# Dicklesworthstone/frankensearch

Hardware: AMD Instinct MI355X
Metric: queries/sec + p50 phase-1 latency, 10M×384 f16 corpus, 1/2/4/8 MI355X (higher is better)
Workload: dtype f16 x f32 -> f32 (every emitted score, in the reference's operation order); candidate filter i8 x i8 -> i32

## Files before the change

### frankensearch_amd/_lib.py

```python
from __future__ import annotations

import ctypes as C
import os

HERE = os.path.dirname(os.path.abspath(__file__))
LIB_PATH = os.path.join(HERE, "libfsgpu.so")

OK = 0
ERR_DIMENSION_MISMATCH = 1
ERR_INVALID_CONFIG = 2
ERR_INDEX_CORRUPTED = 3
ERR_INDEX_VERSION_MISMATCH = 4
ERR_IO = 5
ERR_DEVICE = 6
ERR_NO_DEVICE = 7
ERR_NULL_ARGUMENT = 8
ERR_EMBEDDING_FAILED = 9
ERR_MODEL_LOAD_FAILED = 10

ZERO_SIGNAL_NONE = 0
ZERO_SIGNAL_CALLER_REQUESTED_ZERO_K = 1
ZERO_SIGNAL_ZERO_NORM_QUERY = 2
ZERO_SIGNAL_FILTER_ELIMINATED_ALL = 3
ZERO_SIGNAL_NEWLY_CREATED_EMPTY = 4
# ... 86 lines not shown
    "fsgpu_sharded_search_end": (_i32, [_vp, _u64, _vp, _vp, _vp, _vp]),
    "fsgpu_sharded_quant_scale_max": (C.c_float, [_vp]),
    "fsgpu_sharded_set_coalescing": (_i32, [_vp, _u32, _u32]),
    "fsgpu_sharded_coalescing_stats": (_i32, [_vp, C.POINTER(_u64), C.POINTER(_u64)]),
    "fsgpu_sharded_alignment_create": (_i32, [_vp, _vp, C.POINTER(_vp)]),
    "fsgpu_sharded_quality_scores_for_hits": (_i32, [_vp, _vp, _vp, _vp, _u32, _vp, _u32, _vp, _vp]),
    "fsgpu_sharded_open_fsvi": (_i32, [C.c_char_p, _vp, _u32, _i32, C.POINTER(_vp)]),
    "fsgpu_sharded_set_live_bitmap": (_i32, [_vp, _vp]),
    "fsgpu_sharded_soft_delete": (_i32, [_vp, C.c_char_p, _u32, C.POINTER(_i32)]),
    "fsgpu_sharded_wal_append": (_i32, [_vp, C.c_char_p, _u32, _vp, _u32]),
    "fsgpu_sharded_wal_record_count": (_u64, [_vp]),
    "fsgpu_sharded_doc_id": (_i32, [_vp, _u32, C.POINTER(_vp), C.POINTER(_u32)]),
    "fsgpu_sharded_search_hits": (_i32, [_vp, _vp, _u32, _u32, _vp, _vp, C.POINTER(_u32)]),
    "fsgpu_sharded_gather_dot": (_i32, [_vp, _vp, _u32, _vp, _u32, _vp]),
    "fsgpu_search_topk_classified": (_i32, [_vp, _vp, _u32, _u32, _vp, _vp, C.POINTER(_u32), C.POINTER(_i32)]),
    "fsgpu_search_topk_int8_two_pass": (_i32, [_vp, _vp, _u32, _u32, _u32, _vp, _vp, C.POINTER(_u32)]),
    "fsgpu_search_hits": (_i32, [_vp, _vp, _u32, _u32, _vp, _vp, C.POINTER(_u32)]),
    "fsgpu_search_hits_batched": (_i32, [_vp, _vp, _u32, _u32, _u32, _vp, _vp, _vp, C.POINTER(_u32)]),
    "fsgpu_search_hits_batched_device_queries": (_i32, [_vp, _vp, _u32, _u32, _u32, _vp, _vp, _vp, C.POINTER(_u32)]),
    "fsgpu_search_hits_two_pass_batched": (_i32, [_vp, _vp, _u32, _u32, _u32, _u32, _u32, _vp, _vp, _vp, C.POINTER(_u32)]),
    "fsgpu_lab_index_wal_scores": (_i32, [_vp, _vp, _u32, _vp]),
    "fsgpu_gather_dot": (_i32, [_vp, _vp, _u32, _vp, _u32, _vp]),
    "fsgpu_lab_sort_keys_desc": (_i32, [_i32, _vp, _u64, _u64, _vp]),
    "fsgpu_bench_fixture_device": (_i32, [_i32, _u64, _u64, _u32, _u32, C.c_float, _u64, _i32, _vp, _vp]),
    "fsgpu_encode_f32_to_f16": (_i32, [_i32, _vp, _u64, _vp]),
    "fsgpu_widen_f16_to_f32": (_i32, [_i32, _vp, _u64, _vp]),
    "fsgpu_m2v_create": (_i32, [_i32, _vp, _u32, _u32, C.POINTER(_vp)]),
    "fsgpu_m2v_destroy": (None, [_vp]),
    "fsgpu_m2v_dimension": (_u32, [_vp]),
    "fsgpu_m2v_embed": (_i32, [_vp, _vp, _vp, _u32, _vp]),
    "fsgpu_bert_create": (_i32, [_i32, _vp, _vp, C.POINTER(_vp)]),
    "fsgpu_bert_create_safetensors": (_i32, [_i32, _vp, _u64, C.c_float, C.POINTER(_vp)]),
    "fsgpu_bert_create_ex": (_i32, [_i32, _vp, _vp, _vp, C.POINTER(_vp)]),
    "fsgpu_bert_create_safetensors_ex": (_i32, [_i32, _vp, _u64, C.c_float, _vp, C.POINTER(_vp)]),
    "fsgpu_bert_linear_format": (_u32, [_vp]),
    "fsgpu_lab_linear_int8_dynamic": (_i32, [_i32, _vp, _vp, _vp, _u32, _u32, _u32, _vp]),
    "fsgpu_lab_bert_stage": (_i32, [_i32, _vp]),
    "fsgpu_lab_bert_short_stage": (_i32, [_i32, _vp]),
    "fsgpu_bert_destroy": (None, [_vp]),
    "fsgpu_bert_embed_device": (_i32, [_vp, _vp, _vp, _u32, _vp]),
    "fsgpu_m2v_embed_device": (_i32, [_vp, _vp, _vp, _u32, _vp]),
    "fsgpu_search_topk_batched_device_queries": (_i32, [_vp, _vp, _u32, _u32, _u32, _vp, _vp, _vp, C.POINTER(_u32)]),
    "fsgpu_search_topk_int8_two_pass_batched_device_queries": (_i32, [_vp, _vp, _u32, _u32, _u32, _u32, _vp, _vp, _vp, C.POINTER(_u32)]),
    "fsgpu_device_malloc": (_i32, [_i32, _u64, C.POINTER(_vp)]),
    "fsgpu_device_free": (_i32, [_i32, _vp]),
    "fsgpu_bert_device": (_i32, [_vp]),
# ... 127 lines not shown
```

### frankensearch_amd/csrc/fsgpu_api.cpp

```cpp
#include "../../include/fsgpu.h"
#include "../../include/fsgpu_lab.h"

#include <algorithm>
#include <cmath>
#include <cstring>
#include <exception>
#include <limits>
#include <new>
#include <string>
#include <vector>

#include <atomic>
#include <mutex>
#include <shared_mutex>

#include "bert_embedder.hpp"
#include "bert_reranker.hpp"
#include "coalescer.hpp"
#include "index_builder.hpp"
#include "sharded_index.hpp"
#include "vector_index.hpp"
#include "two_tier_index.hpp"

struct CoalescedCall : fsgpu::CoalescedRequest {
// ... 1625 lines not shown
    return guarded([&]() -> fsgpu_status {
        int count = 0;
        if (hipGetDeviceCount(&count) != hipSuccess || count <= 0) return fail(FSGPU_ERR_NO_DEVICE, "no HIP device visible");
        if (device < 0 || device >= count) return fail(FSGPU_ERR_INVALID_CONFIG, "device ordinal out of range");
        if (hipSetDevice(device) != hipSuccess) return fail(FSGPU_ERR_DEVICE, "hipSetDevice failed");
        if (n == 0) return FSGPU_OK;
        fsgpu::DeviceBuffer in, out, tmp;
        size_t tmp_bytes = 0;
        (void)fsgpu::sort_keys_desc_temp_bytes(n, &tmp_bytes);
        fsgpu::SearchError e = in.reserve(n * 8);
        if (e.ok()) e = out.reserve(n * 8);
        if (e.ok()) e = tmp.reserve(tmp_bytes);
        hipError_t he = hipSuccess;
        if (e.ok()) {
            he = hipMemcpy(in.ptr, keys, n * 8, hipMemcpyHostToDevice);
            if (he == hipSuccess)
                he = fsgpu::sort_keys_desc(tmp.ptr, tmp.bytes, static_cast<const fsgpu::u64*>(in.ptr), static_cast<fsgpu::u64*>(out.ptr), n, nullptr, varying_bits);
            if (he == hipSuccess) he = hipStreamSynchronize(nullptr);
            if (he == hipSuccess) he = hipMemcpy(out_sorted, out.ptr, n * 8, hipMemcpyDeviceToHost);
        }
        in.release();
        out.release();
        tmp.release();
        if (!e.ok()) return finish(e);
        if (he != hipSuccess) return fail(FSGPU_ERR_DEVICE, hipGetErrorString(he));
        return FSGPU_OK;
    });
}

fsgpu_status fsgpu_encode_f32_to_f16(int32_t device, const float* src, uint64_t n, uint16_t* dst) {
    return convert_on_device(device, src, 4, n, dst, 2, true);
}

fsgpu_status fsgpu_widen_f16_to_f32(int32_t device, const uint16_t* src, uint64_t n, float* dst) {
    return convert_on_device(device, src, 2, n, dst, 4, false);
}

fsgpu_status fsgpu_m2v_create(int32_t device, const float* table, uint32_t vocab, uint32_t dim, fsgpu_m2v** out) {
    if (!out) return fail(FSGPU_ERR_NULL_ARGUMENT, "out is null");
    *out = nullptr;
    return guarded([&]() -> fsgpu_status {
        auto* h = new fsgpu_m2v();
        fsgpu::SearchError e = h->impl.init(device, table, vocab, dim);
        if (!e.ok()) {
            delete h;
            return finish(e);
// ... 868 lines not shown
```

### frankensearch_amd/csrc/kernels.hpp

```cpp
#pragma once

#include <hip/hip_runtime.h>
#include <stddef.h>
#include <stdint.h>

namespace fsgpu {

typedef unsigned long long u64;

struct ScanArgs {
    const void* slab;
    const u64* live;
    const u64* allow;
    const float* queries;
    u64* partial;
    uint32_t nrows;
    uint32_t dim;
    uint32_t k;
    uint32_t row_base;
    int32_t hreduce;
    uint32_t row_stride;
};

struct MergeArgs {
// ... 141 lines not shown
constexpr uint32_t kSelectPool = 1024;
constexpr uint32_t kSelectMaxK = 128;
hipError_t launch_select(const SelectArgs& args, int nq, hipStream_t stream);
hipError_t launch_list_cut(const u64* lists, uint32_t nlists, uint32_t list_len, float* out, hipStream_t stream);
hipError_t launch_two_pass_merge(const u64* approx_lists, const u64* exact_lists, uint32_t nshards, uint64_t shard_pitch, uint32_t nq,
                                 uint32_t cc, uint32_t k, uint32_t out_stride, uint32_t* out_rows, float* out_scores, uint32_t* out_counts,
                                 hipStream_t stream);
hipError_t launch_prepare_queries_i8(const float* q, uint32_t nq, uint32_t nq_pad, uint32_t dim, void* qi8, float* delta,
                                     hipStream_t stream, int bits = 8);
hipError_t launch_prepare_queries_i8_filter(const float* q, uint32_t nq, uint32_t nq_pad, uint32_t dim, uint32_t q_stride,
                                            const unsigned int* slab_max_bits, const unsigned int* slab_stats, void* qi8,
                                            float* delta, hipStream_t stream, float* unit_out = nullptr, double extra_coeff = 0.0);

constexpr uint32_t kMfmaMaxSlots = 32;
constexpr uint32_t kMfmaSpillCountStride = 16;
constexpr uint32_t kWideSlots = 32;
bool scan_mfma_supported(int dim);
bool scan_wide_supported(int dim, int elem_bytes);
bool scan_wide_group_maxima_supported(int dim, int query_tiles);
int scan_wide_max_query_tiles(int dim, int elem_bytes);
hipError_t launch_scan_wide(const MfmaScanArgs& args, int query_tiles, int grid, hipStream_t stream, int* occupancy);
void note_main_pass_kernel(const char* name);
const char* last_main_pass_kernel();
int scan_mfma_waves_per_block(int shape);
int scan_mfma_rows_per_tile(int shape);
int scan_mfma_query_tiles(int shape);
int scan_mfma_max_slots(int shape);
hipError_t launch_scan_mfma(const MfmaScanArgs& args, int shape, int grid, hipStream_t stream, int* occupancy);
hipError_t launch_max_row_norm(const void* slab, uint32_t nrows, uint32_t dim, uint32_t row_stride_bytes, unsigned int* out_bits,
                               hipStream_t stream);
hipError_t launch_prepare_queries(const float* q, uint32_t nq, uint32_t nq_pad, uint32_t dim, uint32_t q_stride,
                                  const unsigned int* max_norm_bits, void* qh, float* delta, hipStream_t stream);

hipError_t launch_slab_maxabs(const void* slab_f16, size_t n_values, unsigned int* max_bits_dev, hipStream_t stream);
hipError_t launch_quantize_slab_i8(const void* slab_f16, size_t n_values, unsigned int* max_bits_dev, void* out_i8,
                                   hipStream_t stream, bool max_ready = false);
hipError_t launch_quantize_slab_4bit_levels(const void* slab_f16, size_t n_values, unsigned int* max_bits_dev, void* out_i8,
                                            hipStream_t stream, bool max_ready = false);
hipError_t launch_i8_slab_stats(const void* slab_f16, const void* slab_i8, uint32_t nrows, uint32_t dim,
                                const unsigned int* max_bits_dev, unsigned int* stats_dev, hipStream_t stream);
hipError_t launch_rotate_rows_f16(const void* rows_f16, uint32_t nrows, uint32_t dim, const double* rt, float* out, hipStream_t stream);
hipError_t launch_rotate_rows_f32(const float* rows, uint32_t nrows, uint32_t row_stride, uint32_t dim, const double* rt, float* out,
                                  hipStream_t stream);
hipError_t launch_maxabs_f32(const float* v, size_t n, unsigned int* max_bits_dev, hipStream_t stream);
hipError_t launch_quantize_f32_i8(const float* v, size_t n, const unsigned int* max_bits_dev, void* out_i8, hipStream_t stream);
hipError_t launch_i8_stats_f32(const float* rows, const void* rows_i8, uint32_t nrows, uint32_t dim, const unsigned int* max_bits_dev,
// ... 282 lines not shown
```

### frankensearch_amd/csrc/mfma_scan.hip

```cpp
#include <atomic>
#include <cstdlib>
#include <string>
#include <type_traits>

#include "scan_common.hpp"

namespace fsgpu {

using namespace scan_detail;

typedef float f32x4 __attribute__((ext_vector_type(4)));

template <int DIM_E, int NQT, int WPB, int STAGE, int RT, bool PF, int EB = 2>
__global__ __launch_bounds__(WPB * 64) void scan_mfma_kernel(MfmaScanArgs args) {
    constexpr int DIM = DIM_E * EB / 2;
    typedef int i32x4 __attribute__((ext_vector_type(4)));
    using acc_t = std::conditional_t<EB == 2, f32x4, i32x4>;
    constexpr int NT = WPB * 64;
    constexpr int KS = DIM / 32;
    constexpr int QSTRIDE = DIM + 16;
    constexpr int NQ = NQT * 16;
    extern __shared__ __attribute__((aligned(16))) unsigned char smem[];
    _Float16* qs = reinterpret_cast<_Float16*>(smem);
    const int tid = threadIdx.x, lane = tid & 63;
// ... 256 lines not shown
}
template <int KL>
__device__ __forceinline__ void merge_wave_winners(const u64* win, int k, u64* top, int lane) {
    static_assert(KL == 1, "ranks up to 64");
    if (k <= 16) merge_wave_winners_e<4>(win, k, top, lane);
    else if (k <= 32) merge_wave_winners_e<8>(win, k, top, lane);
    else merge_wave_winners_e<kSelWaves>(win, k, top, lane);
}

constexpr int kSelSortCap = 8192;
constexpr int kRescoreBatch = 6;
constexpr int kSelQueryLds = 1024;
#ifdef FSGPU_EXPERIMENTS
#define SEL_STAMP(slot)                                                                                            \
    do {                                                                                                             \
        if (args.stamps && (blockIdx.x & 255) == 0 && blockIdx.x < 1024 && threadIdx.x == 0)                    \
            args.stamps[(blockIdx.x >> 8) * 16 + (slot)] = (unsigned long long)clock64();                              \
    } while (0)
#else
#define SEL_STAMP(slot) \
    do {                \
    } while (0)
#endif
template <bool FINISH, bool SORTED>
__global__ __launch_bounds__(kSelThreads, SORTED ? 4 : kSelMinWaves) void select_kernel(SelectArgs args) {
    constexpr int NT = kSelThreads, PER = kSelPer, NW = kSelWaves, POOL = (int)kSelectPool, KL = 1;
    static_assert(POOL == NT, "one pool entry per thread in the final selection");
    __shared__ u64 win[2][NW * 64 * KL];
    __shared__ u64 top[64 * KL];
    extern __shared__ __attribute__((aligned(16))) unsigned char sel_dyn[];
    u64* sbuf = reinterpret_cast<u64*>(sel_dyn);
    __shared__ u64 pool[POOL];
    __shared__ int s_count;
    __shared__ float s_tau;
    __shared__ u64 s_gmax[64];
    __shared__ __attribute__((aligned(16))) float s_q[FINISH ? kSelQueryLds : 4];
    __shared__ int s_quick;
    __shared__ u64 s_kth[2];
    const int tid = threadIdx.x, lane = tid & 63, wave = tid >> 6;
    const int q = blockIdx.x;
    SEL_STAMP(0);
    if (args.big_pool && args.pool_flag && args.pool_flag[q] == 0) return;
    auto reset_spill = [&]() {
        if (tid == 0 && args.spill_reset) args.spill_reset[(size_t)q * kMfmaSpillCountStride] = 0u;
    };
    const int k = (int)args.k;
// ... 54 lines not shown
            if (!have) e[x] = kEmpty;
            if (i < lists32) {
                const uint32_t l = i / args.list_len, j = i - l * args.list_len;
                const bool in_list = !cnts || j < (l < kSelCntCap ? s_cnt[l] : cnts[l]);
                if (have && j < kSpecSlots) {
                    if (!in_list) e[x] = kEmpty;
                } else if (in_list) {
                    e[x] = in[(size_t)l * args.l_stride + j];
                } else {
                    e[x] = kEmpty;
                }
            } else if (i < extra_end) {
                e[x] = args.extra[(size_t)q * args.extra_len + (i - lists32)];
            } else if (i < total32) {
                e[x] = args.spill[(size_t)q * args.spill_cap + (i - extra_end)];
            } else {
                e[x] = kEmpty;
            }
        }
    };
    if (tid == 0) s_count = 0;
    pool[tid] = kEmpty;
    int ncand = 0;
    if constexpr (SORTED) {
        __syncthreads();
        for (int p = 0; p < npass; ++p) {
            load_pass(p, e);
#pragma unroll
            for (int x = 0; x < PER; ++x) {
                const bool ok = e[x] != kEmpty;
                const u64 m = __ballot(ok);
                if (m) {
                    int wbase = 0;
                    if (lane == 0) wbase = atomicAdd(&s_count, (int)__popcll(m));
                    wbase = __shfl(wbase, 0);
                    const int pos = wbase + (int)__popcll(m & ((1ull << lane) - 1ull));
                    if (ok && pos < kSelSortCap) sbuf[pos] = e[x];
                }
            }
        }
        __syncthreads();
        int cnt = s_count;
        if (cnt > kSelSortCap) {
            if (tid == 0 && args.overflow) args.overflow[q] = 1;
            cnt = kSelSortCap;
        }
        int np2 = 64;
// ... 466 lines not shown
    if (occupancy) {
        int blocks = 0;
        if (hipOccupancyMaxActiveBlocksPerMultiprocessor(&blocks, kern, WPB * 64, lds) != hipSuccess || blocks < 1) blocks = 1;
        *occupancy = blocks;
        return hipSuccess;
    }
    if (STAGE == 2) {
        static const std::string name = "scan_mfma_kernel<" + std::to_string(DIM) + ", " + std::to_string(NQT) + ", " +
                                        std::to_string(WPB) + ", " + std::to_string(STAGE) + ", " + std::to_string(RT) + ", " +
                                        (PF ? "true" : "false") + ", " + std::to_string(EB) + ">";
        g_last_main_pass_kernel.store(name.c_str(), std::memory_order_relaxed);
    }
    hipLaunchKernelGGL(kern, dim3(grid, args.groups ? args.groups : 1), dim3(WPB * 64), lds, stream, args);
    return hipGetLastError();
}

template <int DIM, int NQT, int WPB, int RT, bool PF, int EB>
static hipError_t launch_mfma_t(const MfmaScanArgs& args, int grid, hipStream_t stream, int* occupancy) {
    if (args.stage == 0) return launch_mfma_s<DIM, NQT, WPB, 0, 1, true, EB>(args, grid, stream, occupancy);
    if (args.stage == 1) return launch_mfma_s<DIM, NQT, WPB, 1, RT, PF, EB>(args, grid, stream, occupancy);
    return launch_mfma_s<DIM, NQT, WPB, 2, RT, PF, EB>(args, grid, stream, occupancy);
}

int scan_mfma_waves_per_block(int shape) { return shape == 0 || shape == 3 ? 4 : 8; }
int scan_mfma_rows_per_tile(int shape) { return shape == 4 ? 64 : (shape >= 2 ? 32 : 16); }
int scan_mfma_query_tiles(int shape) { return shape == 0 ? 4 : (shape == 5 ? 10 : 8); }
int scan_mfma_max_slots(int shape) { return shape == 5 ? 16 : (int)kMfmaMaxSlots; }

template <int DIM, int EB>
static hipError_t launch_mfma_d(const MfmaScanArgs& args, int shape, int grid, hipStream_t stream, int* occupancy) {
    switch (shape) {
        case 0: return launch_mfma_t<DIM, 4, 4, 1, true, EB>(args, grid, stream, occupancy);
        case 2: return launch_mfma_t<DIM, 8, 8, 2, false, EB>(args, grid, stream, occupancy);
#ifdef FSGPU_EXPERIMENTS
        case 1: return launch_mfma_t<DIM, 8, 8, 1, true, EB>(args, grid, stream, occupancy);
        case 3: return launch_mfma_t<DIM, 8, 4, 2, true, EB>(args, grid, stream, occupancy);
        case 4:
            if constexpr (EB == 1) return launch_mfma_t<DIM, 8, 8, 4, false, EB>(args, grid, stream, occupancy);
            return hipErrorInvalidValue;
        case 5: return launch_mfma_t<DIM, 10, 8, 2, false, EB>(args, grid, stream, occupancy);
#endif
        default: return hipErrorInvalidValue;
    }
}

hipError_t launch_scan_mfma(const MfmaScanArgs& args, int shape, int grid, hipStream_t stream, int* occupancy) {
// ... 88 lines not shown
    uint32_t n = 0;
    for (uint32_t j = (uint32_t)tid; j < out_stride; j += 256) {
        const u64 v = j < k && j < (uint32_t)np2 && akey[j] != 0 ? aval[j] : kEmpty;
        if (out_rows) out_rows[(size_t)q * out_stride + j] = (uint32_t)v;
        if (out_scores) out_scores[(size_t)q * out_stride + j] = __uint_as_float((uint32_t)(v >> 32));
    }
    if (tid == 0 && out_counts) {
        const uint32_t lim = k < (uint32_t)np2 ? k : (uint32_t)np2;
        while (n < lim && akey[n] != 0) ++n;
        out_counts[q] = n;
    }
}

hipError_t launch_two_pass_merge(const u64* approx_lists, const u64* exact_lists, uint32_t nshards, uint64_t shard_pitch, uint32_t nq,
                                 uint32_t cc, uint32_t k, uint32_t out_stride, uint32_t* out_rows, float* out_scores, uint32_t* out_counts,
                                 hipStream_t stream) {
    if (nq == 0) return hipSuccess;
    if (cc == 0 || (uint64_t)nshards * cc > 1024 || k > cc) return hipErrorInvalidValue;
    hipLaunchKernelGGL(two_pass_merge_kernel, dim3(nq), dim3(256), 0, stream, approx_lists, exact_lists, nshards, shard_pitch, nq, cc, k,
                       out_stride, out_rows, out_scores, out_counts);
    return hipGetLastError();
}

template <bool RANK, int M, int KCAP>
__global__ __launch_bounds__(512) void select_groups_kernel(GroupSelectArgs args) {
    constexpr int NT = 512, NW = NT / 64, PERT = 1024 / NT, PERW = RANK ? KCAP / 4 : 8, W0 = NW * PERW / 64, NR = M * 8;
    static_assert(NR <= 256 && NR <= NT && NW * PERW % 64 == 0 && W0 >= 1, "W0 winners per lane of wave 0; the rank loop runs on NR threads");
    static_assert(M <= 64 && KCAP >= 64 && KCAP % 64 == 0 && (RANK || M <= NW * PERW), "wave 0 picks M (or k <= KCAP) of the waves' winners");
    __shared__ u64 win[NW * PERW];
    __shared__ u64 top[KCAP];
    __shared__ u64 pool[256];
    __shared__ u64 keys[256];
    __shared__ __attribute__((aligned(16))) float s_q[kSelQueryLds];
    __shared__ u64 s_kth;
    const int tid = threadIdx.x, lane = tid & 63, wave = tid >> 6;
    const int q = blockIdx.x;
    const int k = (int)args.k;
    const float d = args.delta[q];
    const bool real_query = args.valid_queries == 0 || (uint32_t)q < args.valid_queries;
    const int dim = (int)args.dim;
    if (real_query) {
        const float* qsrc = args.queries + (size_t)q * (args.query_stride ? args.query_stride : args.dim);
        for (int i = tid; i < dim && i < kSelQueryLds; i += NT) s_q[i] = qsrc[i];
    }
    u64 e[PERT], key[PERT];
#pragma unroll
    for (int x = 0; x < PERT; ++x) {
        const uint32_t i = (uint32_t)tid + (uint32_t)x * NT;
        e[x] = i < args.nentries ? args.groups[(size_t)q * args.nentries + i] : kEmpty;
        key[x] = e[x] != kEmpty ? sortkey(e[x]) : 0ull;
    }
    if (lane < PERW) win[wave * PERW + lane] = kEmpty;
    if (tid < 256) pool[tid] = kEmpty;
    if (tid == 0) s_kth = 0ull;
    wave_lds_fence();
    wave_extract_topk<PERT>(key, e, PERW, win + wave * PERW);
    __syncthreads();
    if (wave == 0) {
        u64 e2[W0], key2[W0];
#pragma unroll
        for (int x = 0; x < W0; ++x) {
            e2[x] = win[lane + 64 * x];
            key2[x] = e2[x] != kEmpty ? sortkey(e2[x]) : 0ull;
        }
#pragma unroll
        for (int x = 0; x < KCAP / 64; ++x) top[lane + 64 * x] = kEmpty;
        wave_lds_fence();
        wave_extract_topk<W0>(key2, e2, RANK ? (k < KCAP ? k : KCAP) : M, top);
        wave_lds_fence();
    }
    __syncthreads();
    if constexpr (RANK) {
        if (tid == 0) {
            float t = -INFINITY;
            if (d < 0.f || !real_query) {
                t = INFINITY;
                if (args.overflow) args.overflow[q] = 1;
            } else if (k <= KCAP && top[k - 1] != kEmpty) {
                const float ta = __uint_as_float((uint32_t)(top[k - 1] >> 32)) - 2.0f * d;
                if (ta == ta) t = ta;
            }
            args.tau_out[q] = t;
            if (args.spill_reset) args.spill_reset[(size_t)q * kMfmaSpillCountStride] = 0u;
        }
        return;
    }
    for (int c0 = 0; c0 < NR; c0 += NT / 4) {
        const int c = c0 + (tid >> 2), a = tid & 3;
        const int gi = c >> 3, pos = c & 7;
        const u64 ge = c < NR ? top[gi] : kEmpty;
        const uint32_t grow = (uint32_t)ge + (uint32_t)((pos >> 2) * 16 + (pos & 3));
        uint32_t row = grow - args.row_base;
        bool mine = real_query && ge != kEmpty && row < args.nrows && dim <= kSelQueryLds;
        if (mine && args.live) mine = ((args.live[row >> 6] >> (row & 63)) & 1ull) != 0;
        if (mine && args.allow) mine = ((args.allow[row >> 6] >> (row & 63)) & 1ull) != 0;
        if (!mine) row = 0;
        const u32x4* p = reinterpret_cast<const u32x4*>(reinterpret_cast<const unsigned char*>(args.slab) + (size_t)row * ((size_t)dim * 2));
        float acc[8];
#pragma unroll
        for (int j = 0; j < 8; ++j) acc[j] = 0.f;
        const int chunks = dim >> 3, groups = chunks >> 2, leftover = chunks & 3;
        for (int g0 = 0; g0 < groups; g0 += kRescoreBatch) {
            u32x4 w[kRescoreBatch];
#pragma unroll
            for (int j = 0; j < kRescoreBatch; ++j)
                if (g0 + j < groups) w[j] = p[4 * (g0 + j) + a];
#pragma unroll
            for (int j = 0; j < kRescoreBatch; ++j)
                if (g0 + j < groups) {
// ... 33 lines not shown
            if (ak != kEmpty) {
                const float ta = __uint_as_float((uint32_t)(ak >> 32)) - 2.0f * d;
                if (ta == ta) t = ta;
            }
            const u64 kth = s_kth;
            if (kth != 0ull) {
                const float sk = __uint_as_float((uint32_t)(kth >> 32));
                const float v = sk * args.anchor_unit[q];
                const float te = v - d - fabsf(v) * 1e-6f - 1.0f;
                if (te == te && te > t) t = te;
            }
        }
        args.tau_out[q] = t;
        if (args.spill_reset) args.spill_reset[(size_t)q * kMfmaSpillCountStride] = 0u;
    }
}

hipError_t launch_select_groups(const GroupSelectArgs& args, int nq, hipStream_t stream) {
    if (args.k < 1 || args.nentries == 0 || args.nentries > 1024 || !args.delta || !args.tau_out) return hipErrorInvalidValue;
    if (args.rank_only ? args.k > kGroupsRankMax : (args.k > kGroupsTakenMax || (args.dim & 7) || args.dim > kSelQueryLds || !args.anchor_unit || !args.slab))
        return hipErrorInvalidValue;
    constexpr int M0 = (int)kGroupsTaken, M1 = (int)kGroupsTakenMax;
    if (args.rank_only) {
        if (args.k <= 64) hipLaunchKernelGGL((select_groups_kernel<true, M0, 64>), dim3(nq), dim3(512), 0, stream, args);
        else hipLaunchKernelGGL((select_groups_kernel<true, M0, (int)kGroupsRankMax>), dim3(nq), dim3(512), 0, stream, args);
    } else {
        if (args.k <= kGroupsTaken) hipLaunchKernelGGL((select_groups_kernel<false, M0, 64>), dim3(nq), dim3(512), 0, stream, args);
        else hipLaunchKernelGGL((select_groups_kernel<false, M1, 64>), dim3(nq), dim3(512), 0, stream, args);
    }
    return hipGetLastError();
}

__global__ __launch_bounds__(256) void list_cut_kernel(const u64* __restrict__ lists, uint32_t nlists, uint32_t list_len, float* __restrict__ out) {
    __shared__ u64 red[4];
    const int tid = threadIdx.x, lane = tid & 63, wave = tid >> 6;
    u64 m = 0;
    for (uint32_t l = tid; l < nlists; l += 256) {
        const u64 e = lists[(size_t)l * list_len + list_len - 1];
        const u64 key = e != kEmpty ? sortkey(e) : 0ull;
        m = key > m ? key : m;
    }
#pragma unroll
    for (int off = 32; off > 0; off >>= 1) {
        const u64 o = __shfl_xor(m, off);
        m = o > m ? o : m;
    }
    if (lane == 0) red[wave] = m;
    __syncthreads();
    if (tid == 0) {
#pragma unroll
        for (int w = 1; w < 4; ++w) m = red[w] > m ? red[w] : m;
// ... 10 lines not shown
hipError_t launch_select(const SelectArgs& args, int nq, hipStream_t stream) {
    if (args.k < 1 || args.k > kSelectMaxK || !args.delta || (uint64_t)args.nlists * args.list_len > 0x7fffffffull)
        return hipErrorInvalidValue;
#ifdef FSGPU_EXPERIMENTS
    static const int sort_above = [] {
        const char* e = std::getenv("FSGPU_SELECT_SORT_ABOVE");
        return e ? std::atoi(e) : 32;
    }();
#else
    constexpr int sort_above = 32;
#endif
    const bool sorted = (int)args.k > sort_above || args.k > 64 || (args.big_pool && args.slab && !args.take_topk);
    constexpr size_t sort_lds = (size_t)kSelSortCap * 8;
    static bool attr_done = false;
    if (!attr_done) {
        hipError_t e1 = hipFuncSetAttribute(reinterpret_cast<const void*>(select_kernel<true, true>),
                                            hipFuncAttributeMaxDynamicSharedMemorySize, (int)sort_lds);
        hipError_t e2 = hipFuncSetAttribute(reinterpret_cast<const void*>(select_kernel<false, true>),
                                            hipFuncAttributeMaxDynamicSharedMemorySize, (int)sort_lds);
        if (e1 != hipSuccess) return e1;
        if (e2 != hipSuccess) return e2;
        attr_done = true;
    }
    if (args.slab) {
        if (args.k_out < 1 || args.k_out > 64 || (args.dim & 7)) return hipErrorInvalidValue;
        if (sorted) hipLaunchKernelGGL((select_kernel<true, true>), dim3(nq), dim3(kSelThreads), sort_lds, stream, args);
        else hipLaunchKernelGGL((select_kernel<true, false>), dim3(nq), dim3(kSelThreads), 0, stream, args);
    } else {
        if (sorted) hipLaunchKernelGGL((select_kernel<false, true>), dim3(nq), dim3(kSelThreads), sort_lds, stream, args);
        else hipLaunchKernelGGL((select_kernel<false, false>), dim3(nq), dim3(kSelThreads), 0, stream, args);
    }
    return hipGetLastError();
}

hipError_t launch_max_row_norm(const void* slab, uint32_t nrows, uint32_t dim, uint32_t row_stride_bytes, unsigned int* out_bits,
                               hipStream_t stream) {
    hipError_t e = hipMemsetAsync(out_bits, 0, 4, stream);
    if (e != hipSuccess) return e;
    hipLaunchKernelGGL(max_row_norm_kernel, dim3(2048), dim3(256), 0, stream, static_cast<const unsigned short*>(slab),
                       nrows, dim, row_stride_bytes ? row_stride_bytes / 2 : dim, out_bits);
    return hipGetLastError();
}

hipError_t launch_prepare_queries(const float* q, uint32_t nq, uint32_t nq_pad, uint32_t dim, uint32_t q_stride,
                                  const unsigned int* max_norm_bits, void* qh, float* delta, hipStream_t stream) {
    hipLaunchKernelGGL(prepare_queries_kernel, dim3(nq_pad), dim3(256), 0, stream, q, nq, q_stride ? q_stride : dim, dim, max_norm_bits,
                       static_cast<_Float16*>(qh), delta);
    return hipGetLastError();
}

}
```

### frankensearch_amd/csrc/vector_index_batched.cpp

```cpp
#include "vector_index.hpp"

#include <algorithm>
#include <cmath>
#include <cstdio>
#include <cstdlib>
#include <chrono>
#include <cstring>
#include <type_traits>

#include "../../include/fsgpu.h"
#include "lab_env.hpp"
#include "vector_index_internal.hpp"

namespace fsgpu {

using namespace detail;

SearchError VectorIndex::search_top_k_batched_device(const float* queries_dev, uint32_t nq, uint32_t query_len,
                                                     uint32_t k, const uint64_t* allow_dev, uint32_t* out_rows_dev,
                                                     float* out_scores_dev, uint32_t* out_counts_dev,
                                                     hipStream_t stream, uint32_t* fallbacks, uint64_t* out_packed_dev) {
    const bool strided = row_stride_ && row_stride_ != dim_ * 2;
    bool i8f = batched_filter != 1 && (batched_filter == 2 || !i8f_disabled_) && !f32_ && !strided && variant == 0 && knobs().filter != 1 &&
               scan_mfma_supported((int)dim_) && k >= 1 && k <= 64 && nrows_ >= 4 * 8192ull;
// ... 505 lines not shown
        FSGPU_TRY(i8_max_.reserve(4));
        FSGPU_HIP(launch_quantize_slab_i8(slab_dev_, (size_t)nrows_ * dim_, static_cast<unsigned int*>(i8_max_.ptr),
                                          i8_slab_.ptr, stream, quant_max_ready_));
        i8_ready_ = true;
    }
    if (!p.i8 && !mf_norm_ready_) {
        FSGPU_TRY(mf_max_norm_.reserve(4));
        FSGPU_HIP(launch_max_row_norm(slab_dev_, p.N, dim_, p.strided ? row_stride_ : 0, static_cast<unsigned int*>(mf_max_norm_.ptr), stream));
        mf_norm_ready_ = true;
    }
    constexpr uint32_t GMAX = BatchedPlan::GMAX, SPILL = BatchedPlan::SPILL, KC = BatchedPlan::KC;
    const uint32_t round_cap = knobs().round >= (int)GMAX ? (uint32_t)knobs().round : 1024;
    const uint32_t QCAP = std::min<uint32_t>(round_cap, std::max<uint32_t>(std::max<uint32_t>(GMAX, 256), (nq + 127) / 128 * 128));
    p.QCAP = QCAP;
    FSGPU_TRY(mf_qh_.reserve((size_t)QCAP * dim_ * 2));
    FSGPU_TRY(mf_delta_.reserve(QCAP * 4));
    FSGPU_TRY(mf_tau_.reserve(QCAP * 16));
    FSGPU_TRY(mf_spill_.reserve((size_t)QCAP * SPILL * 8 + (size_t)QCAP * kMfmaSpillCountStride * 4));
    FSGPU_TRY(mf_dense_.reserve((size_t)QCAP * RA_MAX * 8));
    FSGPU_TRY(mf_sel_.reserve((size_t)QCAP * KC * 8));
    if (mf_shape_ < 0) {
        mf_shape_ = 2;
        if (knobs().mfma_shape) mf_shape_ = knobs().mfma_shape;
        if (mf_shape_ < 1 || mf_shape_ > 3) mf_shape_ = 2;
        MfmaScanArgs probe{};
        probe.dim = dim_;
        probe.stage = 2;
        FSGPU_HIP(launch_scan_mfma(probe, 0, 1, stream, &mf_per_cu_narrow_));
        FSGPU_HIP(launch_scan_mfma(probe, mf_shape_, 1, stream, &mf_per_cu_wide_));
        probe.elem_bytes = 1;
        mf_shape_i8_ = 2;
        if (knobs().mfma_shape_i8) mf_shape_i8_ = knobs().mfma_shape_i8;
        if (mf_shape_i8_ < 1 || mf_shape_i8_ > 4) mf_shape_i8_ = 2;
        FSGPU_HIP(launch_scan_mfma(probe, 0, 1, stream, &mf_per_cu_narrow_i8_));
        FSGPU_HIP(launch_scan_mfma(probe, mf_shape_i8_, 1, stream, &mf_per_cu_wide_i8_));
        mf_use_160_ = knobs().use_160;
        if (mf_use_160_) {
            FSGPU_HIP(launch_scan_mfma(probe, 5, 1, stream, &mf_per_cu_160_i8_));
            probe.elem_bytes = 2;
            FSGPU_HIP(launch_scan_mfma(probe, 5, 1, stream, &mf_per_cu_160_));
        }
    }
    p.wide_pref = knobs().wide >= 0 ? knobs().wide : 3;
    p.wide_max = (uint32_t)std::max(2, std::min(knobs().wide_max > 0 ? knobs().wide_max : 5, scan_wide_max_query_tiles((int)dim_, p.i8 ? 1 : 2)));
    p.wide_ok = (p.wide_pref == 2 || p.wide_pref == 3) && scan_wide_supported((int)dim_, p.i8 ? 1 : 2) && variant != 5 && variant != 6;
    const uint32_t flag_cap = (nq + GMAX - 1) / GMAX * GMAX + 256;
    if (flag_cap > mf_flags_cap_) {
        if (async_state_[0] == 1 || async_state_[1] == 1)
            return make_error(FSGPU_ERR_INVALID_CONFIG, "a begun batched search is outstanding: end it before searching with a larger batch");
        if (mf_flags_host_) (void)hipHostFree(mf_flags_host_);
        mf_flags_host_ = nullptr;
        mf_flags_cap_ = 0;
        FSGPU_HIP(hipHostMalloc(reinterpret_cast<void**>(&mf_flags_host_), (size_t)flag_cap * 8 * 3, hipHostMallocMapped));
        mf_flags_cap_ = flag_cap;
    }
    uint32_t* flags_area = mf_flags_host_ + (size_t)((async_want_ >= 0 && !hard_batch_) ? 1 + async_want_ : 0) * mf_flags_cap_ * 2;
// ... 663 lines not shown
```

### include/fsgpu_lab.h

```cpp
#ifndef FSGPU_LAB_H
#define FSGPU_LAB_H

#include "fsgpu.h"

#ifdef __cplusplus
extern "C" {
#endif

fsgpu_status fsgpu_bench_fixture_device(int32_t device, uint64_t first, uint64_t n, uint32_t dim, uint32_t clusters, float noise,
                                        uint64_t seed_base, int32_t as_f16, void *out_dev, void *hip_stream);

fsgpu_status fsgpu_index_set_profiling(fsgpu_index *idx, int32_t enabled);
fsgpu_status fsgpu_index_scan_time(fsgpu_index *idx, double *total_ms, uint64_t *launches, int32_t reset);
fsgpu_status fsgpu_index_scan_stats(fsgpu_index *idx, double *total_ms, uint64_t *launches, uint64_t *rows,
                                    int32_t reset);
fsgpu_status fsgpu_index_filter_stats(fsgpu_index *idx, uint64_t *gathered, uint64_t *scanned);
const char *fsgpu_last_main_pass_kernel(void);
fsgpu_status fsgpu_lab_sort_keys_desc(int32_t device, const uint64_t *keys, uint64_t n, uint64_t varying_bits, uint64_t *out_sorted);
fsgpu_status fsgpu_lab_linear_int8_dynamic(int32_t device, const float *x, const float *w, const float *bias, uint32_t m, uint32_t n,
                                           uint32_t k, float *y);
#define FSGPU_LAB_BERT_ATTENTION 0
#define FSGPU_LAB_BERT_LINEAR 1
#define FSGPU_LAB_BERT_LINEAR_LN 2
#define FSGPU_LAB_BERT_POST_ATTN 3
#define FSGPU_LAB_BERT_EMBED_LN 4
#define FSGPU_LAB_BERT_POOL 5
typedef struct fsgpu_lab_bert_stage_args {
    uint32_t stage, form, epilogue;
    uint32_t m, n, k, hidden, inter, n_docs, vocab, max_pos;
    float eps, scale;
    const uint32_t *offsets;
    const int32_t *ids, *positions, *types;
    const float *in[12];
    float *out0, *out1;
} fsgpu_lab_bert_stage_args;
fsgpu_status fsgpu_lab_bert_stage(int32_t device, const fsgpu_lab_bert_stage_args *args);
#define FSGPU_LAB_BERT_Q_ATTN 0
#define FSGPU_LAB_BERT_Q_GEMM 1
#define FSGPU_LAB_BERT_Q_POOL 2
#define FSGPU_LAB_BERT_DOCS 3
typedef struct fsgpu_lab_bert_short_args {
// ... 26 lines not shown
```

Baseline: 366,500.

## Replace sorted top-k selection and group rank threshold with LDS radix select

Adds a byte-wise radix-select path to the sorted select kernel for small candidate sets. It finds the k-th key via 256-bin histograms, compacts the survivors and ranks them, replacing the multi-pass sort and the large dynamic shared-memory allocation. The rank-only group select kernel likewise computes its threshold by radix histogram instead of wave top-k extraction, which removes the KCAP template variant. It also adds a lab test entry point and a guard against MFMA shapes that were not compiled. The trade-off is more barriers and shared-memory atomics in exchange for less sorting work and lower shared-memory use.

```diff
diff --git a/frankensearch_amd/_lib.py b/frankensearch_amd/_lib.py
--- a/frankensearch_amd/_lib.py
+++ b/frankensearch_amd/_lib.py
@@ -132,6 +132,7 @@
     "fsgpu_lab_index_wal_scores": (_i32, [_vp, _vp, _u32, _vp]),
     "fsgpu_gather_dot": (_i32, [_vp, _vp, _u32, _vp, _u32, _vp]),
     "fsgpu_lab_sort_keys_desc": (_i32, [_i32, _vp, _u64, _u64, _vp]),
+    "fsgpu_lab_select_topk": (_i32, [_i32, _vp, _u32, _u32, _u32, _vp]),
     "fsgpu_bench_fixture_device": (_i32, [_i32, _u64, _u64, _u32, _u32, C.c_float, _u64, _i32, _vp, _vp]),
     "fsgpu_encode_f32_to_f16": (_i32, [_i32, _vp, _u64, _vp]),
     "fsgpu_widen_f16_to_f32": (_i32, [_i32, _vp, _u64, _vp]),
diff --git a/frankensearch_amd/csrc/fsgpu_api.cpp b/frankensearch_amd/csrc/fsgpu_api.cpp
--- a/frankensearch_amd/csrc/fsgpu_api.cpp
+++ b/frankensearch_amd/csrc/fsgpu_api.cpp
@@ -1671,6 +1671,48 @@
         in.release();
         out.release();
         tmp.release();
+        if (!e.ok()) return finish(e);
+        if (he != hipSuccess) return fail(FSGPU_ERR_DEVICE, hipGetErrorString(he));
+        return FSGPU_OK;
+    });
+}
+
+fsgpu_status fsgpu_lab_select_topk(int32_t device, const uint64_t* entries, uint32_t nq, uint32_t n, uint32_t k, uint64_t* out) {
+    if (nq && (!out || (n && !entries))) return fail(FSGPU_ERR_NULL_ARGUMENT, "entries / out is null");
+    if (n > 8192 || k < 1 || k > 128) return fail(FSGPU_ERR_INVALID_CONFIG, "n <= 8192, 1 <= k <= 128");
+    return guarded([&]() -> fsgpu_status {
+        int count = 0;
+        if (hipGetDeviceCount(&count) != hipSuccess || count <= 0) return fail(FSGPU_ERR_NO_DEVICE, "no HIP device visible");
+        if (device < 0 || device >= count) return fail(FSGPU_ERR_INVALID_CONFIG, "device ordinal out of range");
+        if (hipSetDevice(device) != hipSuccess) return fail(FSGPU_ERR_DEVICE, "hipSetDevice failed");
+        if (nq == 0) return FSGPU_OK;
+        constexpr size_t POOL = fsgpu::kSelectPool;
+        fsgpu::DeviceBuffer in, pool, delta;
+        fsgpu::SearchError e = in.reserve(std::max<size_t>((size_t)nq * n, 1) * 8);
+        if (e.ok()) e = pool.reserve((size_t)nq * POOL * 8);
+        if (e.ok()) e = delta.reserve((size_t)nq * 4);
+        hipError_t he = hipSuccess;
+        if (e.ok()) {
+            if (n) he = hipMemcpy(in.ptr, entries, (size_t)nq * n * 8, hipMemcpyHostToDevice);
+            if (he == hipSuccess) he = hipMemset(delta.ptr, 0, (size_t)nq * 4);
+            fsgpu::SelectArgs a{};
+            a.lists = static_cast<const fsgpu::u64*>(in.ptr);
+            a.q_stride = n;
+            a.l_stride = n;
+            a.nlists = n ? 1 : 0;
+            a.list_len = n;
+            a.k = k;
+            a.take_topk = 1;
+            a.delta = static_cast<const float*>(delta.ptr);
+            a.pool_out = static_cast<fsgpu::u64*>(pool.ptr);
+            if (he == hipSuccess) he = fsgpu::launch_select(a, (int)nq, nullptr);
+            if (he == hipSuccess) he = hipStreamSynchronize(nullptr);
+            for (uint32_t q = 0; q < nq && he == hipSuccess; ++q)
+                he = hipMemcpy(out + (size_t)q * 128, static_cast<const fsgpu::u64*>(pool.ptr) + (size_t)q * POOL, 128 * 8, hipMemcpyDeviceToHost);
+        }
+        in.release();
+        pool.release();
+        delta.release();
         if (!e.ok()) return finish(e);
         if (he != hipSuccess) return fail(FSGPU_ERR_DEVICE, hipGetErrorString(he));
         return FSGPU_OK;
diff --git a/frankensearch_amd/csrc/kernels.hpp b/frankensearch_amd/csrc/kernels.hpp
--- a/frankensearch_amd/csrc/kernels.hpp
+++ b/frankensearch_amd/csrc/kernels.hpp
@@ -187,6 +187,7 @@
 hipError_t launch_scan_wide(const MfmaScanArgs& args, int query_tiles, int grid, hipStream_t stream, int* occupancy);
 void note_main_pass_kernel(const char* name);
 const char* last_main_pass_kernel();
+bool scan_mfma_shape_compiled(int shape, int elem_bytes);
 int scan_mfma_waves_per_block(int shape);
 int scan_mfma_rows_per_tile(int shape);
 int scan_mfma_query_tiles(int shape);
diff --git a/frankensearch_amd/csrc/mfma_scan.hip b/frankensearch_amd/csrc/mfma_scan.hip
--- a/frankensearch_amd/csrc/mfma_scan.hip
+++ b/frankensearch_amd/csrc/mfma_scan.hip
@@ -302,6 +302,11 @@
     do {                \
     } while (0)
 #endif
+__host__ __device__ inline bool select_radix_topk(const SelectArgs& a) {
+    return a.take_topk && !a.big_pool && !a.tau_out && !a.tau_floor_out && !a.heur_rank &&
+           (uint64_t)a.nlists * a.list_len + a.extra_len + (a.spill ? a.spill_cap : 0u) <= (uint64_t)kSelThreads * kSelPer;
+}
+
 template <bool FINISH, bool SORTED>
 __global__ __launch_bounds__(kSelThreads, SORTED ? 4 : kSelMinWaves) void select_kernel(SelectArgs args) {
     constexpr int NT = kSelThreads, PER = kSelPer, NW = kSelWaves, POOL = (int)kSelectPool, KL = 1;
@@ -402,7 +407,103 @@
     if (tid == 0) s_count = 0;
     pool[tid] = kEmpty;
     int ncand = 0;
-    if constexpr (SORTED) {
+    if (SORTED && select_radix_topk(args)) {
+        __shared__ uint32_t hist[256];
+        __shared__ u64 s_prefix;
+        __shared__ uint32_t s_need, s_stop;
+        __syncthreads();
+        load_pass(0, e);
+        u64 key[PER];
+#pragma unroll
+        for (int x = 0; x < PER; ++x) key[x] = e[x] != kEmpty ? sortkey(e[x]) : 0ull;
+        auto key_of = [&](int x) { return key[x]; };
+        u64 prefix = 0ull, mask = 0ull;
+        uint32_t need = (uint32_t)k;
+#pragma unroll 1
+        for (int shift = 56; shift >= 0; shift -= 8) {
+            if (tid < 256) hist[tid] = 0u;
+            __syncthreads();
+#pragma unroll
+            for (int x = 0; x < PER; ++x) {
+                const u64 kx = key_of(x);
+                if (kx != 0ull && (kx & mask) == prefix) {
+                    const uint32_t bin = (uint32_t)(kx >> shift) & 255u;
+                    const uint32_t first = (uint32_t)__builtin_amdgcn_readfirstlane((int)bin);
+                    const u64 act = __ballot(1);
+                    if (__ballot(bin != first) == 0ull) {
+                        if (lane == (int)__ffsll((long long)act) - 1) atomicAdd(&hist[first], (uint32_t)__popcll(act));
+                    } else {
+                        atomicAdd(&hist[bin], 1u);
+                    }
+                }
+            }
+            __syncthreads();
+            if (wave == 0) {
+                uint32_t h[4], sum = 0;
+#pragma unroll
+                for (int j = 0; j < 4; ++j) {
+                    h[j] = hist[255 - 4 * lane - j];
+                    sum += h[j];
+                }
+                uint32_t incl = sum;
+#pragma unroll
+                for (int off = 1; off < 64; off <<= 1) {
+                    const uint32_t o = __shfl_up(incl, off);
+                    if (lane >= off) incl += o;
+                }
+                uint32_t above = incl - sum;
+                if (lane == 63 && incl < need) s_stop = 2u;
+                if (above < need && need <= incl) {
+#pragma unroll
+                    for (int j = 0; j < 4; ++j) {
+                        if (above < need && need <= above + h[j]) {
+                            s_prefix = prefix | ((u64)(uint32_t)(255 - 4 * lane - j) << shift);
+                            s_need = need - above;
+                            s_stop = need - above == h[j] ? 1u : 0u;
+                        }
+                        above += h[j];
+                    }
+                }
+            }
+            __syncthreads();
+            const uint32_t stop = s_stop;
+            if (stop == 2u) break;
+            prefix = s_prefix;
+            need = s_need;
+            mask |= 255ull << shift;
+            if (stop) break;
+        }
+        if (tid == 0 && dq < 0.f && args.overflow) args.overflow[q] = 1;
+#pragma unroll
+        for (int x = 0; x < PER; ++x) {
+            const u64 kx = key_of(x);
+            const bool ok = kx != 0ull && (kx & mask) >= prefix;
+            const u64 m = __ballot(ok);
+            if (m) {
+                int wbase = 0;
+                if (lane == 0) wbase = atomicAdd(&s_count, (int)__popcll(m));
+                wbase = __shfl(wbase, 0);
+                const int pos = wbase + (int)__popcll(m & ((1ull << lane) - 1ull));
+                if (ok && pos < POOL) pool[pos] = e[x];
+            }
+        }
+        __syncthreads();
+        const int nsel = s_count < POOL ? s_count : POOL;
+        u64* ordered = win[0];
+        if (tid < nsel) {
+            const u64 mine = sortkey(pool[tid]);
+            int greater = 0;
+            for (int j = 0; j < nsel; ++j) {
+                const u64 o = sortkey(pool[j]);
+                greater += (o > mine || (o == mine && j < tid)) ? 1 : 0;
+            }
+            if (greater < k) ordered[greater] = pool[tid];
+        }
+        __syncthreads();
+        ncand = nsel < k ? nsel : k;
+        pool[tid] = tid < ncand ? ordered[tid] : kEmpty;
+        __syncthreads();
+    } else if constexpr (SORTED) {
         __syncthreads();
         for (int p = 0; p < npass; ++p) {
             load_pass(p, e);
@@ -915,6 +1016,14 @@
     return launch_mfma_s<DIM, NQT, WPB, 2, RT, PF, EB>(args, grid, stream, occupancy);
 }
 
+bool scan_mfma_shape_compiled(int shape, int elem_bytes) {
+#ifdef FSGPU_EXPERIMENTS
+    return shape == 0 || shape == 1 || shape == 2 || shape == 3 || shape == 5 || (shape == 4 && elem_bytes == 1);
+#else
+    (void)elem_bytes;
+    return shape == 0 || shape == 2;
+#endif
+}
 int scan_mfma_waves_per_block(int shape) { return shape == 0 || shape == 3 ? 4 : 8; }
 int scan_mfma_rows_per_tile(int shape) { return shape == 4 ? 64 : (shape >= 2 ? 32 : 16); }
 int scan_mfma_query_tiles(int shape) { return shape == 0 ? 4 : (shape == 5 ? 10 : 8); }
@@ -1049,16 +1158,16 @@
     return hipGetLastError();
 }
 
-template <bool RANK, int M, int KCAP>
+template <bool RANK, int M>
 __global__ __launch_bounds__(512) void select_groups_kernel(GroupSelectArgs args) {
-    constexpr int NT = 512, NW = NT / 64, PERT = 1024 / NT, PERW = RANK ? KCAP / 4 : 8, W0 = NW * PERW / 64, NR = M * 8;
+    constexpr int NT = 512, NW = NT / 64, PERT = 1024 / NT, PERW = 8, W0 = NW * PERW / 64, NR = M * 8;
     static_assert(NR <= 256 && NR <= NT && NW * PERW % 64 == 0 && W0 >= 1, "W0 winners per lane of wave 0; the rank loop runs on NR threads");
-    static_assert(M <= 64 && KCAP >= 64 && KCAP % 64 == 0 && (RANK || M <= NW * PERW), "wave 0 picks M (or k <= KCAP) of the waves' winners");
+    static_assert(M <= 64 && M <= NW * PERW, "wave 0 picks M of the waves' winners");
     __shared__ u64 win[NW * PERW];
-    __shared__ u64 top[KCAP];
+    __shared__ u64 top[64];
     __shared__ u64 pool[256];
     __shared__ u64 keys[256];
-    __shared__ __attribute__((aligned(16))) float s_q[kSelQueryLds];
+    __shared__ __attribute__((aligned(16))) float s_q[RANK ? 4 : kSelQueryLds];
     __shared__ u64 s_kth;
     const int tid = threadIdx.x, lane = tid & 63, wave = tid >> 6;
     const int q = blockIdx.x;
@@ -1066,7 +1175,7 @@
     const float d = args.delta[q];
     const bool real_query = args.valid_queries == 0 || (uint32_t)q < args.valid_queries;
     const int dim = (int)args.dim;
-    if (real_query) {
+    if (real_query && !RANK) {
         const float* qsrc = args.queries + (size_t)q * (args.query_stride ? args.query_stride : args.dim);
         for (int i = tid; i < dim && i < kSelQueryLds; i += NT) s_q[i] = qsrc[i];
     }
@@ -1076,6 +1185,70 @@
         const uint32_t i = (uint32_t)tid + (uint32_t)x * NT;
         e[x] = i < args.nentries ? args.groups[(size_t)q * args.nentries + i] : kEmpty;
         key[x] = e[x] != kEmpty ? sortkey(e[x]) : 0ull;
+    }
+    if constexpr (RANK) {
+        __shared__ uint32_t hist[256];
+        __shared__ uint32_t s_sel[2];
+        uint32_t prefix = 0, mask = 0, need = (uint32_t)k;
+        bool found = true;
+#pragma unroll 1
+        for (int shift = 24; shift >= 0; shift -= 8) {
+            if (tid < 256) hist[tid] = 0u;
+            __syncthreads();
+#pragma unroll
+            for (int x = 0; x < PERT; ++x) {
+                const uint32_t o = (uint32_t)(key[x] >> 32);
+                if (key[x] != 0ull && (o & mask) == prefix) atomicAdd(&hist[(o >> shift) & 255u], 1u);
+            }
+            __syncthreads();
+            if (wave == 0) {
+                uint32_t h[4], s = 0;
+#pragma unroll
+                for (int j = 0; j < 4; ++j) {
+                    h[j] = hist[255 - 4 * lane - j];
+                    s += h[j];
+                }
+                uint32_t incl = s;
+#pragma unroll
+                for (int off = 1; off < 64; off <<= 1) {
+                    const uint32_t o = __shfl_up(incl, off);
+                    if (lane >= off) incl += o;
+                }
+                uint32_t above = incl - s;
+                if (lane == 63 && incl < need) s_sel[1] = 0u;
+                if (above < need && need <= incl) {
+#pragma unroll
+                    for (int j = 0; j < 4; ++j) {
+                        if (above < need && need <= above + h[j]) {
+                            s_sel[0] = prefix | ((uint32_t)(255 - 4 * lane - j) << shift);
+                            s_sel[1] = need - above;
+                        }
+                        above += h[j];
+                    }
+                }
+            }
+            __syncthreads();
+            prefix = s_sel[0];
+            need = s_sel[1];
+            mask |= 255u << shift;
+            if (need == 0u) {
+                found = false;
+                break;
+            }
+        }
+        if (tid == 0) {
+            float t = -INFINITY;
+            if (d < 0.f || !real_query) {
+                t = INFINITY;
+                if (args.overflow) args.overflow[q] = 1;
+            } else if (found) {
+                const float ta = __uint_as_float(score_from_sortkey((u64)prefix << 32)) - 2.0f * d;
+                if (ta == ta) t = ta;
+            }
+            args.tau_out[q] = t;
+            if (args.spill_reset) args.spill_reset[(size_t)q * kMfmaSpillCountStride] = 0u;
+        }
+        return;
     }
     if (lane < PERW) win[wave * PERW + lane] = kEmpty;
     if (tid < 256) pool[tid] = kEmpty;
@@ -1090,28 +1263,12 @@
             e2[x] = win[lane + 64 * x];
             key2[x] = e2[x] != kEmpty ? sortkey(e2[x]) : 0ull;
         }
-#pragma unroll
-        for (int x = 0; x < KCAP / 64; ++x) top[lane + 64 * x] = kEmpty;
+        top[lane] = kEmpty;
         wave_lds_fence();
-        wave_extract_topk<W0>(key2, e2, RANK ? (k < KCAP ? k : KCAP) : M, top);
+        wave_extract_topk<W0>(key2, e2, M, top);
         wave_lds_fence();
     }
     __syncthreads();
-    if constexpr (RANK) {
-        if (tid == 0) {
-            float t = -INFINITY;
-            if (d < 0.f || !real_query) {
-                t = INFINITY;
-                if (args.overflow) args.overflow[q] = 1;
-            } else if (k <= KCAP && top[k - 1] != kEmpty) {
-                const float ta = __uint_as_float((uint32_t)(top[k - 1] >> 32)) - 2.0f * d;
-                if (ta == ta) t = ta;
-            }
-            args.tau_out[q] = t;
-            if (args.spill_reset) args.spill_reset[(size_t)q * kMfmaSpillCountStride] = 0u;
-        }
-        return;
-    }
     for (int c0 = 0; c0 < NR; c0 += NT / 4) {
         const int c = c0 + (tid >> 2), a = tid & 3;
         const int gi = c >> 3, pos = c & 7;
@@ -1191,11 +1348,10 @@
         return hipErrorInvalidValue;
     constexpr int M0 = (int)kGroupsTaken, M1 = (int)kGroupsTakenMax;
     if (args.rank_only) {
-        if (args.k <= 64) hipLaunchKernelGGL((select_groups_kernel<true, M0, 64>), dim3(nq), dim3(512), 0, stream, args);
-        else hipLaunchKernelGGL((select_groups_kernel<true, M0, (int)kGroupsRankMax>), dim3(nq), dim3(512), 0, stream, args);
+        hipLaunchKernelGGL((select_groups_kernel<true, M0>), dim3(nq), dim3(512), 0, stream, args);
     } else {
-        if (args.k <= kGroupsTaken) hipLaunchKernelGGL((select_groups_kernel<false, M0, 64>), dim3(nq), dim3(512), 0, stream, args);
-        else hipLaunchKernelGGL((select_groups_kernel<false, M1, 64>), dim3(nq), dim3(512), 0, stream, args);
+        if (args.k <= kGroupsTaken) hipLaunchKernelGGL((select_groups_kernel<false, M0>), dim3(nq), dim3(512), 0, stream, args);
+        else hipLaunchKernelGGL((select_groups_kernel<false, M1>), dim3(nq), dim3(512), 0, stream, args);
     }
     return hipGetLastError();
 }
@@ -1252,12 +1408,13 @@
         if (e2 != hipSuccess) return e2;
         attr_done = true;
     }
+    const size_t sorted_lds = select_radix_topk(args) ? 0 : sort_lds;
     if (args.slab) {
         if (args.k_out < 1 || args.k_out > 64 || (args.dim & 7)) return hipErrorInvalidValue;
-        if (sorted) hipLaunchKernelGGL((select_kernel<true, true>), dim3(nq), dim3(kSelThreads), sort_lds, stream, args);
+        if (sorted) hipLaunchKernelGGL((select_kernel<true, true>), dim3(nq), dim3(kSelThreads), sorted_lds, stream, args);
         else hipLaunchKernelGGL((select_kernel<true, false>), dim3(nq), dim3(kSelThreads), 0, stream, args);
     } else {
-        if (sorted) hipLaunchKernelGGL((select_kernel<false, true>), dim3(nq), dim3(kSelThreads), sort_lds, stream, args);
+        if (sorted) hipLaunchKernelGGL((select_kernel<false, true>), dim3(nq), dim3(kSelThreads), sorted_lds, stream, args);
         else hipLaunchKernelGGL((select_kernel<false, false>), dim3(nq), dim3(kSelThreads), 0, stream, args);
     }
     return hipGetLastError();
diff --git a/frankensearch_amd/csrc/vector_index_batched.cpp b/frankensearch_amd/csrc/vector_index_batched.cpp
--- a/frankensearch_amd/csrc/vector_index_batched.cpp
+++ b/frankensearch_amd/csrc/vector_index_batched.cpp
@@ -551,7 +551,7 @@
     if (mf_shape_ < 0) {
         mf_shape_ = 2;
         if (knobs().mfma_shape) mf_shape_ = knobs().mfma_shape;
-        if (mf_shape_ < 1 || mf_shape_ > 3) mf_shape_ = 2;
+        if (mf_shape_ < 1 || mf_shape_ > 3 || !scan_mfma_shape_compiled(mf_shape_, 2)) mf_shape_ = 2;
         MfmaScanArgs probe{};
         probe.dim = dim_;
         probe.stage = 2;
@@ -560,7 +560,7 @@
         probe.elem_bytes = 1;
         mf_shape_i8_ = 2;
         if (knobs().mfma_shape_i8) mf_shape_i8_ = knobs().mfma_shape_i8;
-        if (mf_shape_i8_ < 1 || mf_shape_i8_ > 4) mf_shape_i8_ = 2;
+        if (mf_shape_i8_ < 1 || mf_shape_i8_ > 4 || !scan_mfma_shape_compiled(mf_shape_i8_, 1)) mf_shape_i8_ = 2;
         FSGPU_HIP(launch_scan_mfma(probe, 0, 1, stream, &mf_per_cu_narrow_i8_));
         FSGPU_HIP(launch_scan_mfma(probe, mf_shape_i8_, 1, stream, &mf_per_cu_wide_i8_));
         mf_use_160_ = knobs().use_160;
diff --git a/include/fsgpu_lab.h b/include/fsgpu_lab.h
--- a/include/fsgpu_lab.h
+++ b/include/fsgpu_lab.h
@@ -17,6 +17,7 @@
 fsgpu_status fsgpu_index_filter_stats(fsgpu_index *idx, uint64_t *gathered, uint64_t *scanned);
 const char *fsgpu_last_main_pass_kernel(void);
 fsgpu_status fsgpu_lab_sort_keys_desc(int32_t device, const uint64_t *keys, uint64_t n, uint64_t varying_bits, uint64_t *out_sorted);
+fsgpu_status fsgpu_lab_select_topk(int32_t device, const uint64_t *entries, uint32_t nq, uint32_t n, uint32_t k, uint64_t *out);
 fsgpu_status fsgpu_lab_linear_int8_dynamic(int32_t device, const float *x, const float *w, const float *bias, uint32_t m, uint32_t n,
                                            uint32_t k, float *y);
 #define FSGPU_LAB_BERT_ATTENTION 0
```

Result: no change. 367,100, median of 2 (+0.2%).
